# Ruyi-Zha/endosurf

Measured on AMD Instinct MI355X. Metric: training rays/sec (1024 rays x 64 samples), higher is better.
Workload: dtype f32

## Files before the change

### endosurf_amd/csrc/chain_common.h

```cpp
#pragma once
#include <hip/hip_runtime.h>

#include "arch.h"

namespace es {

typedef float f32x16 __attribute__((ext_vector_type(16)));

__device__ __forceinline__ float relu1(float z) {
    float r;
    asm("v_max_f32_e32 %0, 0, %1" : "=v"(r) : "v"(z));
    return r;
}

constexpr int TM = 64;
constexpr int NTHREADS = 256;
constexpr int MAIN_FLOATS = HID * TM;
constexpr int AUX56_FLOATS = 56 * TM;
constexpr int LEAN_LDS_BYTES = (MAIN_FLOATS + AUX56_FLOATS + 256) * 4;

__device__ __forceinline__ int swz(int k, int r) { return k * TM + (r ^ ((k & 15) << 2)); }

template <int RTC, int NTC>
__device__ __forceinline__ void acc_zero(f32x16 (&acc)[RTC][NTC]) {
#pragma unroll
    for (int i = 0; i < RTC; ++i)
#pragma unroll
        for (int j = 0; j < NTC; ++j)
#pragma unroll
            for (int r = 0; r < 16; ++r) acc[i][j][r] = 0.f;
}

__device__ __forceinline__ float f4c(const float4& v, int j) { return j == 0 ? v.x : (j == 1 ? v.y : (j == 2 ? v.z : v.w)); }

template <int KG, int RTC, int NTC, int PF = 2>
__device__ __forceinline__ void gemm_seg(f32x16 (&acc)[RTC][NTC], const float* At, const float4* __restrict__ W,
                                         int rt0, int nt0, int lane) {
    static_assert(PF == 2 || PF == 4, "prefetch groups: even-group parity of the swizzle table");
    constexpr bool GUARD = (KG % (2 * PF)) != 0;
    const int lo = lane & 31, hi = lane >> 5;
    float4 b0[PF][NTC], b1[PF][NTC];
    const float4* wl = W + lane;
    int aoff[RTC][8];
#pragma unroll
    for (int ri = 0; ri < RTC; ++ri)
#pragma unroll
        for (int c = 0; c < 8; ++c) aoff[ri][c] = ((((rt0 + ri) * 32 + lo) ^ (hi << 2)) ^ (8 * c)) + 64 * hi;

    auto loadB = [&](float4(&b)[PF][NTC], int g0) {
#pragma unroll
        for (int gi = 0; gi < PF; ++gi)
#pragma unroll
            for (int ni = 0; ni < NTC; ++ni)
                if (!GUARD || g0 + gi < KG) b[gi][ni] = wl[(size_t)((nt0 + ni) * KG + g0 + gi) * 64];
    };
    auto comp = [&](const float4(&b)[PF][NTC], int g0) {
        const float* Ag = At + 512 * g0;
#pragma unroll
        for (int gi = 0; gi < PF; ++gi) {
            if (!GUARD || g0 + gi < KG) {
#pragma unroll
                for (int j = 0; j < 4; ++j) {
                    float a[RTC];
#pragma unroll
                    for (int ri = 0; ri < RTC; ++ri) a[ri] = Ag[aoff[ri][4 * (gi & 1) + j] + 512 * gi + 128 * j];
#pragma unroll
                    for (int ri = 0; ri < RTC; ++ri)
#pragma unroll
                        for (int ni = 0; ni < NTC; ++ni)
                            acc[ri][ni] = __builtin_amdgcn_mfma_f32_32x32x2f32(a[ri], f4c(b[gi][ni], j), acc[ri][ni], 0, 0, 0);
                }
            }
        }
    };

    loadB(b0, 0);
    if constexpr (KG > 2 * PF) {
#pragma unroll 1
        for (int g0 = 0; g0 < KG; g0 += 2 * PF) {
            if (!GUARD || g0 + PF < KG) loadB(b1, g0 + PF);
            comp(b0, g0);
            if (g0 + 2 * PF < KG) loadB(b0, g0 + 2 * PF);
            if (!GUARD || g0 + PF < KG) comp(b1, g0 + PF);
        }
    } else {
        if (PF < KG) loadB(b1, PF);
        comp(b0, 0);
        if (PF < KG) comp(b1, PF);
    }
}

template <int RTC, int NTC, class F>
__device__ __forceinline__ void for_quads(f32x16 (&acc)[RTC][NTC], int rt0, int nt0, int lane, F&& f) {
    const int lo = lane & 31, hi = lane >> 5;
#pragma unroll
    for (int ri = 0; ri < RTC; ++ri)
#pragma unroll
        for (int ni = 0; ni < NTC; ++ni)
#pragma unroll
            for (int q = 0; q < 4; ++q) {
                float v[4] = {acc[ri][ni][4 * q + 0], acc[ri][ni][4 * q + 1], acc[ri][ni][4 * q + 2], acc[ri][ni][4 * q + 3]};
                f((rt0 + ri) * 32 + 8 * q + 4 * hi, (nt0 + ni) * 32 + lo, v);
            }
}

template <int RTC, int NTC, class F>
__device__ __forceinline__ void for_quads_noacc(int rt0, int nt0, int lane, F&& f) {
    const int lo = lane & 31, hi = lane >> 5;
#pragma unroll
    for (int ri = 0; ri < RTC; ++ri)
#pragma unroll
        for (int ni = 0; ni < NTC; ++ni)
#pragma unroll
            for (int q = 0; q < 4; ++q) f((rt0 + ri) * 32 + 8 * q + 4 * hi, (nt0 + ni) * 32 + lo);
}

template <int RTC, int NTC, class F>
__device__ __forceinline__ void for_quads_qi(f32x16 (&acc)[RTC][NTC], int rt0, int nt0, int lane, F&& f) {
    const int lo = lane & 31, hi = lane >> 5;
#pragma unroll
    for (int ri = 0; ri < RTC; ++ri)
#pragma unroll
        for (int ni = 0; ni < NTC; ++ni)
#pragma unroll
            for (int q = 0; q < 4; ++q) {
                float v[4] = {acc[ri][ni][4 * q + 0], acc[ri][ni][4 * q + 1], acc[ri][ni][4 * q + 2], acc[ri][ni][4 * q + 3]};
                f((rt0 + ri) * 32 + 8 * q + 4 * hi, (nt0 + ni) * 32 + lo, v, (ri * NTC + ni) * 4 + q);
            }
}
template <int NI, class F>
__device__ __forceinline__ void for_quads_half(f32x16 (&acc)[2][2], int nt0, int lane, F&& f) {
    const int lo = lane & 31, hi = lane >> 5;
#pragma unroll
    for (int ri = 0; ri < 2; ++ri)
#pragma unroll
        for (int q = 0; q < 4; ++q) {
            float v[4] = {acc[ri][NI][4 * q + 0], acc[ri][NI][4 * q + 1], acc[ri][NI][4 * q + 2], acc[ri][NI][4 * q + 3]};
            f(ri * 32 + 8 * q + 4 * hi, (nt0 + NI) * 32 + lo, v, ri * 4 + q);
        }
}

typedef float f32x2v __attribute__((ext_vector_type(2)));
__device__ __forceinline__ void add_bias4(float (&v)[4], float b) {
    const f32x2v bb = {b, b};
    f32x2v lo = {v[0], v[1]}, hi = {v[2], v[3]};
    lo += bb; hi += bb;
    v[0] = lo[0]; v[1] = lo[1]; v[2] = hi[0]; v[3] = hi[1];
}
__device__ __forceinline__ float keep_if_bit(float v, unsigned w, int k) {
    const int m = __builtin_amdgcn_sbfe((int)w, k, 1);
    return __uint_as_float(__float_as_uint(v) & (unsigned)m);
}
template <int RTC> struct QuadOff { int o[RTC * 4]; };
template <int RTC>
__device__ __forceinline__ QuadOff<RTC> quad_offsets(int rt0, int nt0, int lane) {
    QuadOff<RTC> qo;
    const int lo = lane & 31, hi = lane >> 5;
#pragma unroll
    for (int ri = 0; ri < RTC; ++ri)
#pragma unroll
        for (int q = 0; q < 4; ++q) {
            int v = swz(nt0 * 32 + lo, (rt0 + ri) * 32 + 8 * q + 4 * hi);
            asm volatile("" : "+v"(v));
            qo.o[ri * 4 + q] = v;
        }
    return qo;
}
template <int RTC, int NTC, class F>
__device__ __forceinline__ void for_quads_off(f32x16 (&acc)[RTC][NTC], const QuadOff<RTC>& qo, int rt0, int nt0, int lane, F&& f) {
    const int lo = lane & 31, hi = lane >> 5;
#pragma unroll
    for (int ri = 0; ri < RTC; ++ri)
#pragma unroll
        for (int ni = 0; ni < NTC; ++ni)
#pragma unroll
            for (int q = 0; q < 4; ++q) {
                float v[4] = {acc[ri][ni][4 * q + 0], acc[ri][ni][4 * q + 1], acc[ri][ni][4 * q + 2], acc[ri][ni][4 * q + 3]};
                f((rt0 + ri) * 32 + 8 * q + 4 * hi, (nt0 + ni) * 32 + lo, v, qo.o[ri * 4 + q] + 2048 * ni, ni);
            }
}
__device__ __forceinline__ void lds_store_quad_at(float* At, int off, const float (&v)[4]) {
    *reinterpret_cast<float4*>(At + off) = make_float4(v[0], v[1], v[2], v[3]);
}
__device__ __forceinline__ void lds_store_quad(float* At, int col, int row, const float (&v)[4]) {
    *reinterpret_cast<float4*>(&At[swz(col, row)]) = make_float4(v[0], v[1], v[2], v[3]);
}
__device__ __forceinline__ void lds_load_quad(const float* At, int col, int row, float (&v)[4]) {
    const float4 t = *reinterpret_cast<const float4*>(&At[swz(col, row)]);
    v[0] = t.x; v[1] = t.y; v[2] = t.z; v[3] = t.w;
}
__device__ __forceinline__ void lds_add_quad(float* At, int col, int row, const float (&v)[4]) {
    float4* p = reinterpret_cast<float4*>(&At[swz(col, row)]);
    float4 t = *p;
    t.x += v[0]; t.y += v[1]; t.z += v[2]; t.w += v[3];
    *p = t;
}
__device__ __forceinline__ void g_store_quad(float* __restrict__ base, size_t grow0, int ld, int row, int col, const float (&v)[4]) {
    float* p = base + (grow0 + row) * (size_t)ld + col;
    __builtin_nontemporal_store(v[0], p); __builtin_nontemporal_store(v[1], p + ld);
    __builtin_nontemporal_store(v[2], p + 2 * ld); __builtin_nontemporal_store(v[3], p + 3 * ld);
}
__device__ __forceinline__ void g_load_quad(const float* __restrict__ base, size_t grow0, int ld, int row, int col, float (&v)[4]) {
    const float* p = base + (grow0 + row) * (size_t)ld + col;
    v[0] = __builtin_nontemporal_load(p); v[1] = __builtin_nontemporal_load(p + ld);
    v[2] = __builtin_nontemporal_load(p + 2 * ld); v[3] = __builtin_nontemporal_load(p + 3 * ld);
}

typedef float v4f_frag __attribute__((ext_vector_type(4)));
__device__ __forceinline__ size_t frag_off(size_t grow0, int row, int col) {
    const int ri = row >> 5, q = (row >> 3) & 3, hi = (row >> 2) & 1;
    const int w = col >> 6, ni = (col >> 5) & 1, lo = col & 31;
    return grow0 * 256 + (size_t)(((w * 16 + (ri * 2 + ni) * 4 + q) * 64 + hi * 32 + lo) * 4);
}
__device__ __forceinline__ void g_store_quad_f(float* __restrict__ base, size_t grow0, int row, int col, const float (&v)[4]) {
    const v4f_frag t = {v[0], v[1], v[2], v[3]};
    __builtin_nontemporal_store(t, reinterpret_cast<v4f_frag*>(base + frag_off(grow0, row, col)));
}
__device__ __forceinline__ void g_load_quad_f(const float* __restrict__ base, size_t grow0, int row, int col, float (&v)[4]) {
    const v4f_frag t = __builtin_nontemporal_load(reinterpret_cast<const v4f_frag*>(base + frag_off(grow0, row, col)));
    v[0] = t[0]; v[1] = t[1]; v[2] = t[2]; v[3] = t[3];
}
template <int RTC, int NTC>
__device__ __forceinline__ void prefetch_quads_f(float (&buf)[RTC * NTC * 4][4], const float* __restrict__ base, size_t grow0, int rt0, int nt0,
                                                 int lane) {
    const int lo = lane & 31, hi = lane >> 5;
#pragma unroll
    for (int ri = 0; ri < RTC; ++ri)
#pragma unroll
        for (int ni = 0; ni < NTC; ++ni)
#pragma unroll
            for (int q = 0; q < 4; ++q)
                g_load_quad_f(base, grow0, (rt0 + ri) * 32 + 8 * q + 4 * hi, (nt0 + ni) * 32 + lo, buf[(ri * NTC + ni) * 4 + q]);
}
template <int NI>
__device__ __forceinline__ void prefetch_half_f(float (&buf)[8][4], const float* __restrict__ base, size_t grow0, int nt0, int lane) {
    const int lo = lane & 31, hi = lane >> 5;
#pragma unroll
    for (int ri = 0; ri < 2; ++ri)
#pragma unroll
        for (int q = 0; q < 4; ++q) g_load_quad_f(base, grow0, ri * 32 + 8 * q + 4 * hi, (nt0 + NI) * 32 + lo, buf[ri * 4 + q]);
}

template <int NC>
__device__ __forceinline__ void load_tile(float* At, const float* __restrict__ src, size_t grow0, int ld, int tid) {
    const int r = tid >> 2, c4 = tid & 3;
    const float* p = src + (grow0 + r) * (size_t)ld;
#pragma unroll 4
    for (int jj = 0; jj < NC / 16; ++jj) {
        const int c = 4 * (c4 + 4 * jj);
        const float4 v = *reinterpret_cast<const float4*>(p + c);
        At[swz(c + 0, r)] = v.x; At[swz(c + 1, r)] = v.y; At[swz(c + 2, r)] = v.z; At[swz(c + 3, r)] = v.w;
    }
}
__device__ __forceinline__ void load_tile_256(float* At, const float* __restrict__ src, size_t grow0, int ld, int tid) {
    load_tile<256>(At, src, grow0, ld, tid);
}

struct MaskWords { unsigned w[2][2]; };
__device__ __forceinline__ MaskWords load_mask_words(const unsigned* __restrict__ Ml, int tile64, int wave, int lane) {
    MaskWords m;
    const unsigned* p = Ml + (size_t)(2 * tile64) * 256 + wave * 64 + (lane & 31);
    m.w[0][0] = p[0]; m.w[0][1] = p[32]; m.w[1][0] = p[256]; m.w[1][1] = p[256 + 32];
    return m;
}
__device__ __forceinline__ float mask_keep(float v, const MaskWords& m, int qi, int i, int hi) {
    const int ri_c = qi >> 3, ni = (qi >> 2) & 1, q_c = qi & 3;
    const int pq = ((q_c >> 1) * 2 + ni) * 4 + 2 * (q_c & 1) + hi;
    return keep_if_bit(v, m.w[ri_c][i >> 1], 2 * pq + (i & 1));
}
__device__ __forceinline__ bool mask_bit(const MaskWords& m, int qi, int i, int hi) {
    const int ri_c = qi >> 3, ni = (qi >> 2) & 1, q_c = qi & 3;
    const int pq = ((q_c >> 1) * 2 + ni) * 4 + 2 * (q_c & 1) + hi;
    return (m.w[ri_c][i >> 1] >> (2 * pq + (i & 1))) & 1u;
}

__device__ __forceinline__ float softplus100(float z) {
    const float e = __builtin_amdgcn_exp2f(-144.26950408889634f * fabsf(z));
    return fmaf(0.006931471805599453f, __builtin_amdgcn_logf(1.f + e), relu1(z));
}
__device__ __forceinline__ float softplus100_grad_from_s(float s) {
    const float x = 100.f * s;
    return x < 0.02f ? x * (1.f - x * (0.5f - x * (1.f / 6.f))) : 1.f - __expf(-x);
}

typedef float f32x2p __attribute__((ext_vector_type(2)));
__device__ __forceinline__ f32x2p softplus100_grad_from_s2(f32x2p s) {
    const f32x2p x = s * 100.f;
    const f32x2p t = x * -1.4426950408889634f;
    f32x2p e;
    e[0] = __builtin_amdgcn_exp2f(t[0]); e[1] = __builtin_amdgcn_exp2f(t[1]);
    const f32x2p big = 1.f - e;
    const f32x2p ser = x * (1.f - x * (0.5f - x * (1.f / 6.f)));
    f32x2p r;
    r[0] = x[0] < 0.02f ? ser[0] : big[0];
    r[1] = x[1] < 0.02f ? ser[1] : big[1];
    return r;
}
__device__ __forceinline__ void softplus100_grad_from_s4(const float (&s)[4], float (&d)[4]) {
    const f32x2p a = softplus100_grad_from_s2(f32x2p{s[0], s[1]}), b = softplus100_grad_from_s2(f32x2p{s[2], s[3]});
    d[0] = a[0]; d[1] = a[1]; d[2] = b[0]; d[3] = b[1];
}

__device__ __forceinline__ int enc_index(int D, int i, int fn, int c) { return D + (2 * i + fn) * D + c; }

template <int NOUT>
__device__ __forceinline__ void smalln_partial(const float* At, const float* __restrict__ Wrows, int ldw, float* scr, int tid) {
    const int row = tid & 63;
    const int part = __builtin_amdgcn_readfirstlane(tid >> 6);
    float s[NOUT];
#pragma unroll
    for (int i = 0; i < NOUT; ++i) s[i] = 0.f;
    const int k0 = part * 64;
#pragma unroll 8
    for (int kk = 0; kk < 64; ++kk) {
        const float a = At[swz(k0 + kk, row)];
#pragma unroll
        for (int i = 0; i < NOUT; ++i) s[i] = fmaf(Wrows[i * ldw + k0 + kk], a, s[i]);
    }
#pragma unroll
    for (int i = 0; i < NOUT; ++i) scr[(part * NOUT + i) * 64 + row] = s[i];
}
template <int NOUT>
__device__ __forceinline__ float smalln_reduce(const float* scr, int i, int row) {
    return (scr[(0 * NOUT + i) * 64 + row] + scr[(1 * NOUT + i) * 64 + row]) + (scr[(2 * NOUT + i) * 64 + row] + scr[(3 * NOUT + i) * 64 + row]);
}

struct PointSrc {
    const float* x;
    const float* t;
    const float* dirs;
    const float* rays;
    const float* z;
    int mode, t_scalar, n_per_ray, ldz;
    int M, M_split;
};
__device__ __forceinline__ void load_point(const PointSrc& s, int i_in, float (&x)[3], float& t, float (&d)[3]) {
    int i = i_in;
    if (i >= s.M) { x[0] = x[1] = x[2] = 0.f; t = 0.f; d[0] = d[1] = 0.f; d[2] = 1.f; return; }
    if (s.mode == 0 || (s.mode == 2 && i >= s.M_split)) {
        if (s.mode == 2) i -= s.M_split;
        x[0] = s.x[3 * (size_t)i]; x[1] = s.x[3 * (size_t)i + 1]; x[2] = s.x[3 * (size_t)i + 2];
        t = s.t[s.t_scalar ? 0 : i];
        if (s.dirs) { d[0] = s.dirs[3 * (size_t)i]; d[1] = s.dirs[3 * (size_t)i + 1]; d[2] = s.dirs[3 * (size_t)i + 2]; }
        else { d[0] = d[1] = 0.f; d[2] = 1.f; }
    } else {
        const int ray = i / s.n_per_ray, smp = i - ray * s.n_per_ray;
        const float* r = s.rays + 9 * (size_t)ray;
        const float zz = s.z[(size_t)ray * s.ldz + smp];
        const float inv = r[5] + 1e-6f;
        d[0] = r[3]; d[1] = r[4]; d[2] = r[5];
        x[0] = r[0] + (r[3] / inv) * zz; x[1] = r[1] + (r[4] / inv) * zz; x[2] = r[2] + (r[5] / inv) * zz;
        t = r[8];
    }
}

}
```

### endosurf_amd/csrc/point_bwd.hip

```cpp
#include <type_traits>

#include "chain_common.h"
#include "encode.h"
#include "launch.h"
#include "tabs.h"
#include "timing.h"
#include "workspace.h"
#include "point_bwd_bodies.h"

namespace es {

#ifdef ES_PROFILE_BWD
__device__ long long b_prof[256];
extern "C" int es_debug_b_profile(long long* out, int n) { return (int)hipMemcpyFromSymbol(out, HIP_SYMBOL(b_prof), sizeof(long long) * (n < 256 ? n : 256)); }
#endif

enum BwdBody { BB_NONE = 0, BB_COLOR, BB_SDF, BB_DEFORM, BB_TAN, BB_TAN_SDF, BB_DEFORM_HALF };
template <int B>
__device__ __forceinline__ void bwd_body(const BwdArgs& a, int tile) {
    if constexpr (B == BB_COLOR) color_bwd_tile(a, tile);
    else if constexpr (B == BB_SDF) sdf_bwd_tile(a, tile);
    else if constexpr (B == BB_DEFORM) deform_bwd_tile(a, tile);
    else if constexpr (B == BB_DEFORM_HALF) deform_bwd_tile<true>(a, tile);
    else if constexpr (B == BB_TAN) deform_tan_tile(a, tile);
    else if constexpr (B == BB_TAN_SDF) {
        deform_tan_tile(a, tile);
        __syncthreads();
        sdf_bwd_tile(a, tile);
    }
}
template <int B0, int B1>
__global__ __launch_bounds__(NTHREADS, 2) void k_point_bwd(BwdArgs a, int n0, int t0, int t1) {
    if constexpr (B0 != BB_NONE) {
        if ((int)blockIdx.x < n0) { bwd_body<B0>(a, t0 + blockIdx.x); return; }
    }
    bwd_body<B1>(a, t1 + (int)blockIdx.x - n0);
}
constexpr int bwd_lds(int b) {
    return b == BB_COLOR ? CBWD_LDS_BYTES : (b == BB_SDF ? SBWD_LDS_BYTES : (b == BB_DEFORM || b == BB_DEFORM_HALF ? DBWD_LDS_BYTES : (b == BB_TAN || b == BB_TAN_SDF ? LEAN_LDS_BYTES : 0)));
}
template <int B0, int B1>
static int launch_bwd(const BwdArgs& a, int n0, int t0, int n1, int t1, hipStream_t st) {
    constexpr int lds = bwd_lds(B0) > bwd_lds(B1) ? bwd_lds(B0) : bwd_lds(B1);
    static DeviceOnce attr_done;
    if (attr_done.first()) {
        if (int e = allow_big_lds(k_point_bwd<B0, B1>, lds)) return e;
        attr_done.done();
    }
    if (n0 + n1 <= 0) return ST_OK;
    hipLaunchKernelGGL((k_point_bwd<B0, B1>), dim3(n0 + n1), dim3(NTHREADS), lds, st, a, n0, t0, t1);
    return ST_OK;
}

int deform_tan_x3r(const PointSrc& src, const void* packed_r, const float* weff, float* ws, const WsLayout& L, const float* d_go, hipStream_t st, int m_rows = 0);
int deform_bwd_x3r_with_tail(const BwdArgs& ba, const void* packed_r, int m_main, hipStream_t st);
int color_bwd_x3r(const PointSrc& src, const void* packed_r, const float* weff, float* ws, const WsLayout& L, bool deform, int m_color, const float* d_rgb,
                  hipStream_t st);
int deform_bwd_x3r(const void* packed_r, const float* weff, float* ws, const WsLayout& L, int M, int m_color, hipStream_t st);
const void* packed_x3r_part(const void* packed_x3);

int point_backward_chains(const PointSrc& src, const float* packed, const float* weff, float* ws, int flags, int m_color,
                          const float* d_sdf, const float* d_go, const float* d_rgb, hipStream_t st, const void* packed_x3) {
    if (src.M <= 0) return ST_OK;
    BwdArgs a;
    a.src = src; a.tb = make_tabs(); a.packed = reinterpret_cast<const float4*>(packed); a.weff = weff; a.ws = ws;
    a.L = ws_layout(src.M, flags); a.flags = flags; a.d_sdf = d_sdf; a.d_go = d_go; a.d_rgb = d_rgb;
    a.M_color = (flags & PF_COLOR) ? (m_color > 0 ? m_color : src.M) : 0;
    const int Mp = a.L.Mp, Mcp = round_up64(a.M_color);
    const bool deform = flags & PF_DEFORM;
    if (flags & PF_X3_CHAIN) {
        if (!packed_x3) return fail(ST_BAD_ARG, "point_backward_chains", "PF_X3_CHAIN needs the split weights (es_pack_x3)");
        const void* pr = packed_x3r_part(packed_x3);
        if (deform && aux_tail(flags, a.M_color, src.M) && a.M_color % 128 == 0) {
            const int Mc = a.M_color;
            if (int e = color_bwd_x3r(src, pr, weff, ws, a.L, deform, Mc, d_rgb, st)) return e;
            if (int e = deform_tan_x3r(src, pr, weff, ws, a.L, d_go, st, Mc)) return e;
            { ScopedTimer tm(KID_SDF_BWD, Mc, st); if (int e = launch_bwd<BB_NONE, BB_SDF>(a, 0, 0, Mc / TM, 0, st)) return e; }
            if (int e = deform_bwd_x3r_with_tail(a, pr, Mc, st)) return e;
            { ScopedTimer tm(KID_DEFORM_BWD, Mp - Mc, st); if (int e = launch_bwd<BB_NONE, BB_DEFORM_HALF>(a, 0, 0, (Mp - Mc) / 16, Mc / 16, st)) return e; }
            return hip_last("point_backward_chains");
        }
        if (flags & PF_COLOR) { if (int e = color_bwd_x3r(src, pr, weff, ws, a.L, deform, a.M_color, d_rgb, st)) return e; }
        if (deform) { if (int e = deform_tan_x3r(src, pr, weff, ws, a.L, d_go, st)) return e; }
        { ScopedTimer tm(KID_SDF_BWD, src.M, st); if (int e = launch_bwd<BB_NONE, BB_SDF>(a, 0, 0, Mp / TM, 0, st)) return e; }
        if (deform) { if (int e = deform_bwd_x3r(pr, weff, ws, a.L, src.M, a.M_color, st)) return e; }
        return hip_last("point_backward_chains");
    }
    if (deform && aux_tail(flags, a.M_color, src.M)) {
        const int Mc = a.M_color;
        { ScopedTimer tm(KID_COLOR_BWD, Mc, st); if (int e = launch_bwd<BB_NONE, BB_COLOR>(a, 0, 0, Mc / TM, 0, st)) return e; }
        { ScopedTimer tm(KID_DEFORM_TAN, Mc, st); if (int e = launch_bwd<BB_NONE, BB_TAN>(a, 0, 0, Mc / TM, 0, st)) return e; }
        { ScopedTimer tm(KID_SDF_BWD, Mc, st); if (int e = launch_bwd<BB_NONE, BB_SDF>(a, 0, 0, Mc / TM, 0, st)) return e; }
        { ScopedTimer tm(KID_DEFORM_BWD, src.M, st);
          if (int e = launch_bwd<BB_TAN_SDF, BB_DEFORM>(a, (Mp - Mc) / TM, Mc / TM, Mc / 32, 0, st)) return e;
          if (int e = launch_bwd<BB_NONE, BB_DEFORM_HALF>(a, 0, 0, (Mp - Mc) / 16, Mc / 16, st)) return e; }
        return hip_last("point_backward_chains");
    }
    if (!deform && aux_tail(flags, a.M_color, src.M)) {
        const int Mc = a.M_color;
        { ScopedTimer tm(KID_COLOR_BWD, Mc, st); if (int e = launch_bwd<BB_SDF, BB_COLOR>(a, (Mp - Mc) / TM, Mc / TM, Mc / TM, 0, st)) return e; }
        { ScopedTimer tm(KID_SDF_BWD, Mc, st); if (int e = launch_bwd<BB_NONE, BB_SDF>(a, 0, 0, Mc / TM, 0, st)) return e; }
        return hip_last("point_backward_chains");
    }
    if (deform) { ScopedTimer tm(KID_DEFORM_TAN, src.M, st); if (int e = launch_bwd<BB_NONE, BB_TAN>(a, 0, 0, Mp / TM, 0, st)) return e; }
    if (flags & PF_COLOR) { ScopedTimer tm(KID_COLOR_BWD, a.M_color, st); if (int e = launch_bwd<BB_NONE, BB_COLOR>(a, 0, 0, Mcp / TM, 0, st)) return e; }
    { ScopedTimer tm(KID_SDF_BWD, src.M, st); if (int e = launch_bwd<BB_NONE, BB_SDF>(a, 0, 0, Mp / TM, 0, st)) return e; }
    if (deform) { ScopedTimer tm(KID_DEFORM_BWD, src.M, st); if (int e = launch_bwd<BB_NONE, BB_DEFORM>(a, 0, 0, Mp / 32, 0, st)) return e; }
    return hip_last("point_backward_chains");
}

}
```

### endosurf_amd/csrc/point_fwd.hip

```cpp
#include "chain_common.h"
#include "encode.h"
#include "launch.h"
#include "tabs.h"
#include "timing.h"
#include "workspace.h"
#include "point_fwd_bodies.h"

namespace es {

enum FwdBody { FB_NONE = 0, FB_DEFORM, FB_SDF, FB_COLOR, FB_VJP, FB_SDF_VJP, FB_DEFORM_HALF, FB_SDF_VJP_HALF, FB_SDF_HALF };
template <int B>
__device__ __forceinline__ void fwd_body(const FwdArgs& a, int tile) {
    if constexpr (B == FB_DEFORM) deform_fwd_tile(a, tile);
    else if constexpr (B == FB_DEFORM_HALF) deform_fwd_tile<true>(a, tile);
    else if constexpr (B == FB_SDF) sdf_fwd_tile(a, tile);
    else if constexpr (B == FB_COLOR) color_fwd_tile(a, tile);
    else if constexpr (B == FB_VJP) deform_vjp_tile(a, tile);
    else if constexpr (B == FB_SDF_VJP) {
        sdf_fwd_tile(a, tile);
        __syncthreads();
        deform_vjp_tile(a, tile);
    } else if constexpr (B == FB_SDF_VJP_HALF) {
        sdf_fwd_tile<true>(a, tile);
        __syncthreads();
        deform_vjp_tile<true>(a, tile);
    } else if constexpr (B == FB_SDF_HALF) sdf_fwd_tile<true>(a, tile);
}
template <int B0, int B1>
__global__ __launch_bounds__(NTHREADS, 2) void k_point_fwd(FwdArgs a, int n0, int t0, int t1) {
    if constexpr (B0 != FB_NONE) {
        if ((int)blockIdx.x < n0) { fwd_body<B0>(a, t0 + blockIdx.x); return; }
    }
    fwd_body<B1>(a, t1 + (int)blockIdx.x - n0);
}
constexpr int fwd_lds(int b) { return b == FB_COLOR ? CFWD_LDS_BYTES : (b == FB_NONE ? 0 : LEAN_LDS_BYTES); }
template <int B0, int B1>
static int launch_fwd(const FwdArgs& a, int n0, int t0, int n1, int t1, hipStream_t st) {
    constexpr int lds = fwd_lds(B0) > fwd_lds(B1) ? fwd_lds(B0) : fwd_lds(B1);
    static DeviceOnce attr_done;
    if (attr_done.first()) {
        if (int e = allow_big_lds(k_point_fwd<B0, B1>, lds)) return e;
        attr_done.done();
    }
    if (n0 + n1 <= 0) return ST_OK;
    hipLaunchKernelGGL((k_point_fwd<B0, B1>), dim3(n0 + n1), dim3(NTHREADS), lds, st, a, n0, t0, t1);
    return ST_OK;
}

int deform_jvp_x3r(const PointSrc& src, const void* packed_r, const float* weff, float* ws, const WsLayout& L, bool save, hipStream_t st);
int deform_vjp_x3r(const PointSrc& src, const void* packed_r, const float* weff, float* ws, const WsLayout& L, bool save, hipStream_t st, int m_rows = 0);
int deform_jvp_x3r_with_tail(const FwdArgs& fa, const void* packed_r, int m_main, hipStream_t st);
int sdf_fwd_x3r(const PointSrc& src, const void* packed_r, const float* weff, float* ws, const WsLayout& L, bool deform, bool color, hipStream_t st);
int color_fwd_x3r(const PointSrc& src, const void* packed_r, const float* weff, float* ws, const WsLayout& L, bool deform, int Mcp, bool save, hipStream_t st);
const void* packed_x3r_part(const void* packed_x3);

int point_forward(const PointSrc& src, const float* packed, const float* weff, float* ws, int flags, int m_color, hipStream_t st,
                  const void* packed_x3) {
    if (src.M <= 0) return ST_OK;
    FwdArgs a;
    a.src = src; a.tb = make_tabs(); a.packed = reinterpret_cast<const float4*>(packed); a.weff = weff; a.ws = ws;
    a.L = ws_layout(src.M, flags); a.flags = flags;
    a.M_color = (flags & PF_COLOR) ? (m_color > 0 ? m_color : src.M) : 0;
    const int Mp = a.L.Mp, Mcp = round_up64(a.M_color);
    const bool deform = flags & PF_DEFORM;
    if ((flags & PF_X3) && !(flags & PF_SAVE) && packed_x3) {
        const void* pr = packed_x3r_part(packed_x3);
        if (deform) { if (int e = deform_jvp_x3r(src, pr, weff, ws, a.L, false, st)) return e; }
        if (int e = sdf_fwd_x3r(src, pr, weff, ws, a.L, deform, (flags & PF_COLOR) != 0, st)) return e;
        if (flags & PF_COLOR) { if (int e = color_fwd_x3r(src, pr, weff, ws, a.L, deform, Mcp, false, st)) return e; }
        return deform ? deform_vjp_x3r(src, pr, weff, ws, a.L, false, st) : hip_last("point_forward");
    }
    if ((flags & PF_X3_CHAIN) && (flags & PF_SAVE) && packed_x3) {
        const void* pr = packed_x3r_part(packed_x3);
        if (deform && aux_tail(flags, a.M_color, src.M) && a.M_color % 128 == 0) {
            const int Mc = a.M_color;
            { ScopedTimer tm(KID_DEFORM_FWD, Mp - Mc, st); if (int e = launch_fwd<FB_NONE, FB_DEFORM_HALF>(a, 0, 0, (Mp - Mc) / 16, Mc / 16, st)) return e; }
            if (int e = deform_jvp_x3r_with_tail(a, pr, Mc, st)) return e;
            { ScopedTimer tm(KID_SDF_FWD, Mc, st); if (int e = launch_fwd<FB_NONE, FB_SDF>(a, 0, 0, Mc / TM, 0, st)) return e; }
            if (int e = color_fwd_x3r(src, pr, weff, ws, a.L, deform, Mc, true, st)) return e;
            return deform_vjp_x3r(src, pr, weff, ws, a.L, true, st, Mc);
        }
        if (deform) { if (int e = deform_jvp_x3r(src, pr, weff, ws, a.L, true, st)) return e; }
        { ScopedTimer tm(KID_SDF_FWD, src.M, st); if (int e = launch_fwd<FB_NONE, FB_SDF>(a, 0, 0, Mp / TM, 0, st)) return e; }
        if (flags & PF_COLOR) { if (int e = color_fwd_x3r(src, pr, weff, ws, a.L, deform, Mcp, true, st)) return e; }
        return deform ? deform_vjp_x3r(src, pr, weff, ws, a.L, true, st) : hip_last("point_forward");
    }
    if (deform && aux_tail(flags, a.M_color, src.M)) {
        const int Mc = a.M_color;
        { ScopedTimer tm(KID_DEFORM_FWD, src.M, st);
          if (int e = launch_fwd<FB_NONE, FB_DEFORM_HALF>(a, 0, 0, (Mp - Mc) / 16, Mc / 16, st)) return e;
          if (int e = launch_fwd<FB_SDF_VJP, FB_DEFORM>(a, (Mp - Mc) / TM, Mc / TM, Mc / 32, 0, st)) return e; }
        { ScopedTimer tm(KID_SDF_FWD, Mc, st); if (int e = launch_fwd<FB_NONE, FB_SDF>(a, 0, 0, Mc / TM, 0, st)) return e; }
        { ScopedTimer tm(KID_COLOR_FWD, Mc, st); if (int e = launch_fwd<FB_NONE, FB_COLOR>(a, 0, 0, Mc / TM, 0, st)) return e; }
        { ScopedTimer tm(KID_DEFORM_VJP, Mc, st); if (int e = launch_fwd<FB_NONE, FB_VJP>(a, 0, 0, Mc / TM, 0, st)) return e; }
        return hip_last("point_forward");
    }
    if (!deform && aux_tail(flags, a.M_color, src.M)) {
        const int Mc = a.M_color;
        { ScopedTimer tm(KID_SDF_FWD, Mc, st); if (int e = launch_fwd<FB_NONE, FB_SDF>(a, 0, 0, Mc / TM, 0, st)) return e; }
        { ScopedTimer tm(KID_COLOR_FWD, Mc, st); if (int e = launch_fwd<FB_SDF, FB_COLOR>(a, (Mp - Mc) / TM, Mc / TM, Mc / TM, 0, st)) return e; }
        return hip_last("point_forward");
    }
    if (deform) { ScopedTimer tm(KID_DEFORM_FWD, src.M, st); if (int e = launch_fwd<FB_NONE, FB_DEFORM>(a, 0, 0, Mp / 32, 0, st)) return e; }
    { ScopedTimer tm(KID_SDF_FWD, src.M, st); if (int e = launch_fwd<FB_NONE, FB_SDF>(a, 0, 0, Mp / TM, 0, st)) return e; }
    if (flags & PF_COLOR) { ScopedTimer tm(KID_COLOR_FWD, a.M_color, st); if (int e = launch_fwd<FB_NONE, FB_COLOR>(a, 0, 0, Mcp / TM, 0, st)) return e; }
    if (deform) { ScopedTimer tm(KID_DEFORM_VJP, src.M, st); if (int e = launch_fwd<FB_NONE, FB_VJP>(a, 0, 0, Mp / TM, 0, st)) return e; }
    return hip_last("point_forward");
}


int point_forward_rows(const PointSrc& src, const float* packed, const float* weff, float* ws, int flags, int m_color, int row0, int nrows,
                       hipStream_t st) {
    if (src.M <= 0 || nrows <= 0) return ST_OK;
    FwdArgs a;
    a.src = src; a.tb = make_tabs(); a.packed = reinterpret_cast<const float4*>(packed); a.weff = weff; a.ws = ws;
    a.L = ws_layout(src.M, flags); a.flags = flags;
    a.M_color = (flags & PF_COLOR) ? (m_color > 0 ? m_color : src.M) : 0;
    const int Mc = a.M_color;
    const bool deform = flags & PF_DEFORM;
    if (row0 + nrows > a.L.Mp) return fail(ST_BAD_ARG, "point_forward_rows", "rows beyond the workspace");
    if (row0 == 0 && nrows == Mc && Mc % 64 == 0) {
        if (deform) { ScopedTimer tm(KID_DEFORM_FWD, Mc, st); if (int e = launch_fwd<FB_NONE, FB_DEFORM>(a, 0, 0, Mc / 32, 0, st)) return e; }
        { ScopedTimer tm(KID_SDF_FWD, Mc, st); if (int e = launch_fwd<FB_NONE, FB_SDF>(a, 0, 0, Mc / TM, 0, st)) return e; }
        { ScopedTimer tm(KID_COLOR_FWD, Mc, st); if (int e = launch_fwd<FB_NONE, FB_COLOR>(a, 0, 0, Mc / TM, 0, st)) return e; }
        if (deform) { ScopedTimer tm(KID_DEFORM_VJP, Mc, st); if (int e = launch_fwd<FB_NONE, FB_VJP>(a, 0, 0, Mc / TM, 0, st)) return e; }
        return hip_last("point_forward_rows");
    }
    if (row0 < Mc || row0 % 64 != 0 || nrows % 64 != 0)
        return fail(ST_BAD_ARG, "point_forward_rows", "rows: either the whole colour part [0, m_color) or a 64-aligned piece of the colour-less tail");
    if (deform) {
        { ScopedTimer tm(KID_DEFORM_FWD, nrows, st); if (int e = launch_fwd<FB_NONE, FB_DEFORM_HALF>(a, 0, 0, nrows / 16, row0 / 16, st)) return e; }
        { ScopedTimer tm(KID_SDF_FWD, nrows, st); if (int e = launch_fwd<FB_NONE, FB_SDF_VJP_HALF>(a, 0, 0, nrows / 32, row0 / 32, st)) return e; }
    } else {
        ScopedTimer tm(KID_SDF_FWD, nrows, st);
        if (int e = launch_fwd<FB_NONE, FB_SDF_HALF>(a, 0, 0, nrows / 32, row0 / 32, st)) return e;
    }
    return hip_last("point_forward_rows");
}

int point_vjp(const PointSrc& src, const float* packed, const float* weff, float* ws, int flags, hipStream_t st) {
    if (src.M <= 0) return ST_OK;
    FwdArgs a;
    a.src = src; a.tb = make_tabs(); a.packed = reinterpret_cast<const float4*>(packed); a.weff = weff; a.ws = ws;
    a.L = ws_layout(src.M, flags); a.flags = flags & ~PF_SAVE;
    a.M_color = 0;
    ScopedTimer tm(KID_DEFORM_VJP, src.M, st);
    if (int e = launch_fwd<FB_NONE, FB_VJP>(a, 0, 0, a.L.Mp / TM, 0, st)) return e;
    return hip_last("point_vjp");
}

int color_forward(const PointSrc& src, const float* packed, const float* weff, float* ws, hipStream_t st) {
    if (src.M <= 0) return ST_OK;
    FwdArgs a;
    a.src = src; a.tb = make_tabs(); a.packed = reinterpret_cast<const float4*>(packed); a.weff = weff; a.ws = ws;
    a.flags = PF_COLOR | PF_RAW_DIR;
    a.L = ws_layout(src.M, PF_COLOR); a.M_color = src.M;
    ScopedTimer tm(KID_COLOR_FWD, src.M, st);
    if (int e = launch_fwd<FB_NONE, FB_COLOR>(a, 0, 0, a.L.Mp / TM, 0, st)) return e;
    return hip_last("color_forward");
}

}
```

### endosurf_amd/csrc/timing.h

```cpp
#pragma once
#include <hip/hip_runtime.h>

namespace es {

enum KernelId : int {
    KID_QUERY = 0, KID_DEFORM_FWD, KID_SDF_FWD, KID_COLOR_FWD, KID_COLOR_BWD, KID_SDF_BWD, KID_DEFORM_BWD,
    KID_WGRAD_D, KID_WGRAD_S, KID_WGRAD_C, KID_WGRAD_SMALL, KID_QUERY_EXIT, KID_DEFORM_VJP, KID_DEFORM_TAN, KID_QUERY16, KID_QUERY_X3, KID_WGRAD_D_X3, KID_WGRAD_S_X3, KID_WGRAD_C_X3,
    KID_DEFORM_FWD_X3, KID_SDF_FWD_X3, KID_COLOR_FWD_X3, KID_DEFORM_VJP_X3,
    KID_DEFORM_TAN_X3, KID_DEFORM_BWD_X3, KID_COLOR_BWD_X3, KID_SDF_BWD_X3, KID_COUNT
};

void timing_begin(int kid, long long rows, hipStream_t st);
void timing_end(int kid, hipStream_t st);

struct ScopedTimer {
    int kid; hipStream_t st;
    ScopedTimer(int k, long long rows, hipStream_t s) : kid(k), st(s) { timing_begin(k, rows, s); }
    ~ScopedTimer() { timing_end(kid, st); }
};

}
```

### endosurf_amd/csrc/timing.hip

```cpp
#include "timing.h"

#include <vector>

#include "../../include/endosurf_hip.h"
#include "device_table.h"
#include "launch.h"

namespace es {

struct TimedLaunch { int kid; long long rows; hipEvent_t a, b; };
struct TimingState {
    bool on = false;
    std::vector<TimedLaunch> launches;
    std::vector<hipEvent_t> pool;
};
static DeviceTable<TimingState> g_timing;
static int g_any_on = 0;

static TimingState& cur_state() {
    int dev = 0;
    if (hipGetDevice(&dev) != hipSuccess) dev = 0;
    return g_timing.at(dev);
}
static hipEvent_t get_event(TimingState& s) {
    if (!s.pool.empty()) { hipEvent_t e = s.pool.back(); s.pool.pop_back(); return e; }
    hipEvent_t e;
    if (hipEventCreate(&e) != hipSuccess) return nullptr;
    return e;
}

void timing_begin(int kid, long long rows, hipStream_t st) {
    if (!g_any_on) return;
    TimingState& s = cur_state();
    if (!s.on) return;
    TimedLaunch t{kid, rows, get_event(s), get_event(s)};
    if (!t.a || !t.b) return;
    hipEventRecord(t.a, st);
    s.launches.push_back(t);
}
void timing_end(int kid, hipStream_t st) {
    if (!g_any_on) return;
    TimingState& s = cur_state();
    if (!s.on || s.launches.empty()) return;
    TimedLaunch& t = s.launches.back();
    if (t.kid == kid) hipEventRecord(t.b, st);
}

}

using namespace es;

extern "C" {

int es_timing_enable(int on) {
    TimingState& s = cur_state();
    const bool want = on != 0;
    if (want != s.on) g_any_on += want ? 1 : -1;
    s.on = want;
    return ST_OK;
}

int es_timing_drain(int capacity, int* kid, long long* rows, float* ms, int* n_out) {
    int n = 0;
    TimingState& s = cur_state();
    auto& g_launches = s.launches;
    auto& g_pool = s.pool;
    for (auto& t : g_launches) {
        float v = 0.f;
        if (hipEventSynchronize(t.b) == hipSuccess && hipEventElapsedTime(&v, t.a, t.b) == hipSuccess && n < capacity) {
            kid[n] = t.kid; rows[n] = t.rows; ms[n] = v; ++n;
        }
        g_pool.push_back(t.a); g_pool.push_back(t.b);
    }
    g_launches.clear();
    if (n_out) *n_out = n;
    (void)hipGetLastError();
    return ST_OK;
}

const char* es_kernel_name(int kid) {
    static const char* names[KID_COUNT] = {"k_query_sdf", "k_deform_fwd", "k_sdf_fwd", "k_color_fwd", "k_color_bwd", "k_sdf_bwd",
                                           "k_deform_bwd", "k_wgrad[deform]", "k_wgrad[sdf]", "k_wgrad[color]", "k_wgrad_small",
                                           "k_query_sdf[later marching blocks: tiles of finished rays exit]", "k_deform_vjp", "k_deform_tan", "k_query_sdf16", "k_query_sdf_x3", "k_wgrad_x3[deform]", "k_wgrad_x3[sdf]", "k_wgrad_x3[color]",
                                           "k_deform_fwd_x3", "k_sdf_fwd_x3", "k_color_fwd_x3", "k_deform_vjp_x3",
                                           "k_deform_tan_x3", "k_deform_bwd_x3", "k_color_bwd_x3", "k_sdf_bwd_x3"};
    return kid >= 0 && kid < KID_COUNT ? names[kid] : "?";
}

}
```

Measured before the change: 72520.

## Fuse per-tile color, deform-tangent and SDF stages into single point kernels

```diff
diff --git a/endosurf_amd/csrc/chain_common.h b/endosurf_amd/csrc/chain_common.h
--- a/endosurf_amd/csrc/chain_common.h
+++ b/endosurf_amd/csrc/chain_common.h
@@ -18,6 +18,11 @@
 constexpr int MAIN_FLOATS = HID * TM;
 constexpr int AUX56_FLOATS = 56 * TM;
 constexpr int LEAN_LDS_BYTES = (MAIN_FLOATS + AUX56_FLOATS + 256) * 4;
+
+__device__ __forceinline__ void stage_handoff() {
+    asm volatile("s_waitcnt vmcnt(0)" ::: "memory");
+    __syncthreads();
+}
 
 __device__ __forceinline__ int swz(int k, int r) { return k * TM + (r ^ ((k & 15) << 2)); }
 
diff --git a/endosurf_amd/csrc/point_bwd.hip b/endosurf_amd/csrc/point_bwd.hip
--- a/endosurf_amd/csrc/point_bwd.hip
+++ b/endosurf_amd/csrc/point_bwd.hip
@@ -15,7 +15,7 @@
 extern "C" int es_debug_b_profile(long long* out, int n) { return (int)hipMemcpyFromSymbol(out, HIP_SYMBOL(b_prof), sizeof(long long) * (n < 256 ? n : 256)); }
 #endif
 
-enum BwdBody { BB_NONE = 0, BB_COLOR, BB_SDF, BB_DEFORM, BB_TAN, BB_TAN_SDF, BB_DEFORM_HALF };
+enum BwdBody { BB_NONE = 0, BB_COLOR, BB_SDF, BB_DEFORM, BB_TAN, BB_TAN_SDF, BB_DEFORM_HALF, BB_COLOR_TAN_SDF };
 template <int B>
 __device__ __forceinline__ void bwd_body(const BwdArgs& a, int tile) {
     if constexpr (B == BB_COLOR) color_bwd_tile(a, tile);
@@ -25,7 +25,17 @@
     else if constexpr (B == BB_TAN) deform_tan_tile(a, tile);
     else if constexpr (B == BB_TAN_SDF) {
         deform_tan_tile(a, tile);
-        __syncthreads();
+        stage_handoff();
+        sdf_bwd_tile(a, tile);
+    } else if constexpr (B == BB_COLOR_TAN_SDF) {
+        if ((a.flags & PF_COLOR) && tile * TM < a.M_color) {
+            color_bwd_tile(a, tile);
+            stage_handoff();
+        }
+        if (a.flags & PF_DEFORM) {
+            deform_tan_tile(a, tile);
+            stage_handoff();
+        }
         sdf_bwd_tile(a, tile);
     }
 }
@@ -37,7 +47,7 @@
     bwd_body<B1>(a, t1 + (int)blockIdx.x - n0);
 }
 constexpr int bwd_lds(int b) {
-    return b == BB_COLOR ? CBWD_LDS_BYTES : (b == BB_SDF ? SBWD_LDS_BYTES : (b == BB_DEFORM || b == BB_DEFORM_HALF ? DBWD_LDS_BYTES : (b == BB_TAN || b == BB_TAN_SDF ? LEAN_LDS_BYTES : 0)));
+    return b == BB_COLOR ? CBWD_LDS_BYTES : (b == BB_SDF ? SBWD_LDS_BYTES : (b == BB_DEFORM || b == BB_DEFORM_HALF ? DBWD_LDS_BYTES : (b == BB_TAN || b == BB_TAN_SDF || b == BB_COLOR_TAN_SDF ? LEAN_LDS_BYTES : 0)));
 }
 template <int B0, int B1>
 static int launch_bwd(const BwdArgs& a, int n0, int t0, int n1, int t1, hipStream_t st) {
@@ -88,9 +98,13 @@
     }
     if (deform && aux_tail(flags, a.M_color, src.M)) {
         const int Mc = a.M_color;
-        { ScopedTimer tm(KID_COLOR_BWD, Mc, st); if (int e = launch_bwd<BB_NONE, BB_COLOR>(a, 0, 0, Mc / TM, 0, st)) return e; }
-        { ScopedTimer tm(KID_DEFORM_TAN, Mc, st); if (int e = launch_bwd<BB_NONE, BB_TAN>(a, 0, 0, Mc / TM, 0, st)) return e; }
-        { ScopedTimer tm(KID_SDF_BWD, Mc, st); if (int e = launch_bwd<BB_NONE, BB_SDF>(a, 0, 0, Mc / TM, 0, st)) return e; }
+        if (!timing_on()) {
+            if (int e = launch_bwd<BB_NONE, BB_COLOR_TAN_SDF>(a, 0, 0, Mc / TM, 0, st)) return e;
+        } else {
+            { ScopedTimer tm(KID_COLOR_BWD, Mc, st); if (int e = launch_bwd<BB_NONE, BB_COLOR>(a, 0, 0, Mc / TM, 0, st)) return e; }
+            { ScopedTimer tm(KID_DEFORM_TAN, Mc, st); if (int e = launch_bwd<BB_NONE, BB_TAN>(a, 0, 0, Mc / TM, 0, st)) return e; }
+            { ScopedTimer tm(KID_SDF_BWD, Mc, st); if (int e = launch_bwd<BB_NONE, BB_SDF>(a, 0, 0, Mc / TM, 0, st)) return e; }
+        }
         { ScopedTimer tm(KID_DEFORM_BWD, src.M, st);
           if (int e = launch_bwd<BB_TAN_SDF, BB_DEFORM>(a, (Mp - Mc) / TM, Mc / TM, Mc / 32, 0, st)) return e;
           if (int e = launch_bwd<BB_NONE, BB_DEFORM_HALF>(a, 0, 0, (Mp - Mc) / 16, Mc / 16, st)) return e; }
@@ -102,9 +116,13 @@
         { ScopedTimer tm(KID_SDF_BWD, Mc, st); if (int e = launch_bwd<BB_NONE, BB_SDF>(a, 0, 0, Mc / TM, 0, st)) return e; }
         return hip_last("point_backward_chains");
     }
-    if (deform) { ScopedTimer tm(KID_DEFORM_TAN, src.M, st); if (int e = launch_bwd<BB_NONE, BB_TAN>(a, 0, 0, Mp / TM, 0, st)) return e; }
-    if (flags & PF_COLOR) { ScopedTimer tm(KID_COLOR_BWD, a.M_color, st); if (int e = launch_bwd<BB_NONE, BB_COLOR>(a, 0, 0, Mcp / TM, 0, st)) return e; }
-    { ScopedTimer tm(KID_SDF_BWD, src.M, st); if (int e = launch_bwd<BB_NONE, BB_SDF>(a, 0, 0, Mp / TM, 0, st)) return e; }
+    if (!timing_on()) {
+        if (int e = launch_bwd<BB_NONE, BB_COLOR_TAN_SDF>(a, 0, 0, Mp / TM, 0, st)) return e;
+    } else {
+        if (deform) { ScopedTimer tm(KID_DEFORM_TAN, src.M, st); if (int e = launch_bwd<BB_NONE, BB_TAN>(a, 0, 0, Mp / TM, 0, st)) return e; }
+        if (flags & PF_COLOR) { ScopedTimer tm(KID_COLOR_BWD, a.M_color, st); if (int e = launch_bwd<BB_NONE, BB_COLOR>(a, 0, 0, Mcp / TM, 0, st)) return e; }
+        { ScopedTimer tm(KID_SDF_BWD, src.M, st); if (int e = launch_bwd<BB_NONE, BB_SDF>(a, 0, 0, Mp / TM, 0, st)) return e; }
+    }
     if (deform) { ScopedTimer tm(KID_DEFORM_BWD, src.M, st); if (int e = launch_bwd<BB_NONE, BB_DEFORM>(a, 0, 0, Mp / 32, 0, st)) return e; }
     return hip_last("point_backward_chains");
 }
diff --git a/endosurf_amd/csrc/point_fwd.hip b/endosurf_amd/csrc/point_fwd.hip
--- a/endosurf_amd/csrc/point_fwd.hip
+++ b/endosurf_amd/csrc/point_fwd.hip
@@ -8,7 +8,7 @@
 
 namespace es {
 
-enum FwdBody { FB_NONE = 0, FB_DEFORM, FB_SDF, FB_COLOR, FB_VJP, FB_SDF_VJP, FB_DEFORM_HALF, FB_SDF_VJP_HALF, FB_SDF_HALF };
+enum FwdBody { FB_NONE = 0, FB_DEFORM, FB_SDF, FB_COLOR, FB_VJP, FB_SDF_VJP, FB_DEFORM_HALF, FB_SDF_VJP_HALF, FB_SDF_HALF, FB_SDF_COLOR_VJP };
 template <int B>
 __device__ __forceinline__ void fwd_body(const FwdArgs& a, int tile) {
     if constexpr (B == FB_DEFORM) deform_fwd_tile(a, tile);
@@ -18,13 +18,24 @@
     else if constexpr (B == FB_VJP) deform_vjp_tile(a, tile);
     else if constexpr (B == FB_SDF_VJP) {
         sdf_fwd_tile(a, tile);
-        __syncthreads();
+        stage_handoff();
         deform_vjp_tile(a, tile);
     } else if constexpr (B == FB_SDF_VJP_HALF) {
         sdf_fwd_tile<true>(a, tile);
-        __syncthreads();
+        stage_handoff();
         deform_vjp_tile<true>(a, tile);
     } else if constexpr (B == FB_SDF_HALF) sdf_fwd_tile<true>(a, tile);
+    else if constexpr (B == FB_SDF_COLOR_VJP) {
+        sdf_fwd_tile(a, tile);
+        if ((a.flags & PF_COLOR) && tile * TM < a.M_color) {
+            stage_handoff();
+            color_fwd_tile(a, tile);
+        }
+        if (a.flags & PF_DEFORM) {
+            stage_handoff();
+            deform_vjp_tile(a, tile);
+        }
+    }
 }
 template <int B0, int B1>
 __global__ __launch_bounds__(NTHREADS, 2) void k_point_fwd(FwdArgs a, int n0, int t0, int t1) {
@@ -90,6 +101,10 @@
         { ScopedTimer tm(KID_DEFORM_FWD, src.M, st);
           if (int e = launch_fwd<FB_NONE, FB_DEFORM_HALF>(a, 0, 0, (Mp - Mc) / 16, Mc / 16, st)) return e;
           if (int e = launch_fwd<FB_SDF_VJP, FB_DEFORM>(a, (Mp - Mc) / TM, Mc / TM, Mc / 32, 0, st)) return e; }
+        if (!timing_on()) {
+            if (int e = launch_fwd<FB_NONE, FB_SDF_COLOR_VJP>(a, 0, 0, Mc / TM, 0, st)) return e;
+            return hip_last("point_forward");
+        }
         { ScopedTimer tm(KID_SDF_FWD, Mc, st); if (int e = launch_fwd<FB_NONE, FB_SDF>(a, 0, 0, Mc / TM, 0, st)) return e; }
         { ScopedTimer tm(KID_COLOR_FWD, Mc, st); if (int e = launch_fwd<FB_NONE, FB_COLOR>(a, 0, 0, Mc / TM, 0, st)) return e; }
         { ScopedTimer tm(KID_DEFORM_VJP, Mc, st); if (int e = launch_fwd<FB_NONE, FB_VJP>(a, 0, 0, Mc / TM, 0, st)) return e; }
@@ -99,6 +114,11 @@
         const int Mc = a.M_color;
         { ScopedTimer tm(KID_SDF_FWD, Mc, st); if (int e = launch_fwd<FB_NONE, FB_SDF>(a, 0, 0, Mc / TM, 0, st)) return e; }
         { ScopedTimer tm(KID_COLOR_FWD, Mc, st); if (int e = launch_fwd<FB_SDF, FB_COLOR>(a, (Mp - Mc) / TM, Mc / TM, Mc / TM, 0, st)) return e; }
+        return hip_last("point_forward");
+    }
+    if (!timing_on()) {
+        if (deform) { if (int e = launch_fwd<FB_NONE, FB_DEFORM>(a, 0, 0, Mp / 32, 0, st)) return e; }
+        if (int e = launch_fwd<FB_NONE, FB_SDF_COLOR_VJP>(a, 0, 0, Mp / TM, 0, st)) return e;
         return hip_last("point_forward");
     }
     if (deform) { ScopedTimer tm(KID_DEFORM_FWD, src.M, st); if (int e = launch_fwd<FB_NONE, FB_DEFORM>(a, 0, 0, Mp / 32, 0, st)) return e; }
@@ -121,6 +141,10 @@
     if (row0 + nrows > a.L.Mp) return fail(ST_BAD_ARG, "point_forward_rows", "rows beyond the workspace");
     if (row0 == 0 && nrows == Mc && Mc % 64 == 0) {
         if (deform) { ScopedTimer tm(KID_DEFORM_FWD, Mc, st); if (int e = launch_fwd<FB_NONE, FB_DEFORM>(a, 0, 0, Mc / 32, 0, st)) return e; }
+        if (!timing_on()) {
+            if (int e = launch_fwd<FB_NONE, FB_SDF_COLOR_VJP>(a, 0, 0, Mc / TM, 0, st)) return e;
+            return hip_last("point_forward_rows");
+        }
         { ScopedTimer tm(KID_SDF_FWD, Mc, st); if (int e = launch_fwd<FB_NONE, FB_SDF>(a, 0, 0, Mc / TM, 0, st)) return e; }
         { ScopedTimer tm(KID_COLOR_FWD, Mc, st); if (int e = launch_fwd<FB_NONE, FB_COLOR>(a, 0, 0, Mc / TM, 0, st)) return e; }
         if (deform) { ScopedTimer tm(KID_DEFORM_VJP, Mc, st); if (int e = launch_fwd<FB_NONE, FB_VJP>(a, 0, 0, Mc / TM, 0, st)) return e; }
diff --git a/endosurf_amd/csrc/timing.h b/endosurf_amd/csrc/timing.h
--- a/endosurf_amd/csrc/timing.h
+++ b/endosurf_amd/csrc/timing.h
@@ -11,6 +11,7 @@
 };
 
 void timing_begin(int kid, long long rows, hipStream_t st);
+bool timing_on();
 void timing_end(int kid, hipStream_t st);
 
 struct ScopedTimer {
diff --git a/endosurf_amd/csrc/timing.hip b/endosurf_amd/csrc/timing.hip
--- a/endosurf_amd/csrc/timing.hip
+++ b/endosurf_amd/csrc/timing.hip
@@ -28,6 +28,8 @@
     if (hipEventCreate(&e) != hipSuccess) return nullptr;
     return e;
 }
+
+bool timing_on() { return g_any_on && cur_state().on; }
 
 void timing_begin(int kid, long long rows, hipStream_t st) {
     if (!g_any_on) return;
```

Result: no change. 72690, median of 6 (+0.2%).
